# jrobine/actor-critic

Hardware: AMD Instinct MI355X
Metric: env-steps/sec (whole node) + ACKTR update ms, Breakout 84x84x4 (higher is better)
Workload: dtype fp32

## Files before the change

actor-critic_amd/csrc/convt2.hpp:

```cpp
#pragma once

#include "f16x2.hpp"
#include "gemm.hpp"

namespace acmi {

struct CT2 {
  static constexpr int CIN = 32, COUT = 64, OH = 9, OW = 9, PW = 10, L = 100;
  static constexpr int NKS = 16;
  static constexpr int STEP_BYTES = 4 * 2 * 1024;
  static constexpr int FRAG_BYTES = NKS * STEP_BYTES;
  static constexpr int BYTES = FRAG_BYTES + 4 * kAmaxWords;
  static constexpr int TILE = 128;
};

__device__ __forceinline__ void convt2_wmax_body(const float* w2, char* out, int b, int nb) {
  float m = 0.f;
  for (int i = b * 256 + threadIdx.x; i < 16 * CT2::CIN * CT2::COUT; i += nb * 256)
    m = fmaxf(m, fabsf(w2[i]));
  m = wave_max(m);
  if ((threadIdx.x & 63) == 0) amax_update(reinterpret_cast<unsigned*>(out + CT2::FRAG_BYTES), m);
}

__device__ __forceinline__ void convt2_prep_body(const float* w2, char* out, int blk) {
  const int g = blk * 256 + threadIdx.x;
  if (g >= CT2::NKS * 4 * 64) return;
  const int lane = g & 63, ph = (g >> 6) & 3, ks = g >> 8;
  const int py = ph >> 1, px = ph & 1, t = ks >> 2, a = t >> 1, b = t & 1;
  const int kh = py + 2 * a, kw = px + 2 * b;
  const int ci = lane & 31, co = 16 * (ks & 3) + 8 * (lane >> 5);
  const float* p = w2 + ((kh * 4 + kw) * CT2::CIN + ci) * CT2::COUT + co;
  const float sw = f16x2_scale_of_bits(reinterpret_cast<const unsigned*>(out + CT2::FRAG_BYTES));
  uint4 h, l;
  split2(p[0], p[1], sw, h.x, l.x);
  split2(p[2], p[3], sw, h.y, l.y);
  split2(p[4], p[5], sw, h.z, l.z);
  split2(p[6], p[7], sw, h.w, l.w);
  uint4* d = reinterpret_cast<uint4*>(out + (long long)ks * CT2::STEP_BYTES + ph * 2 * 1024) + lane;
  d[0] = h;
  d[64] = l;
}

template <bool GRAM, bool MASK = false, bool MIX = false>
__global__ __launch_bounds__(256) __attribute__((amdgpu_waves_per_eu(3)))
void convt2_kernel(const char* prep, const float* __restrict__ d2, const float* __restrict__ a1,
                   float* __restrict__ d1, int B, float* __restrict__ gpart, const unsigned* d2max,
                   unsigned* d1max, const float* __restrict__ d2b = nullptr, const unsigned* d2bmax = nullptr) {
  __shared__ __attribute__((aligned(16))) char lds[std::max(2 * CT2::STEP_BYTES, 4 * 32 * 36 * 4)];
  const int tid = threadIdx.x, lane = tid & 63, wave = tid >> 6;
  const int J = B * CT2::L;
  const int ctiles = (J + CT2::TILE - 1) / CT2::TILE;
  const int G = gridDim.x;
  const int gbase = MIX ? (ctiles + G - 1) / G * G : ctiles;
  const int ntiles = MIX ? gbase + ctiles : ctiles;
  auto valid_from = [&](int t) { return MIX && t >= ctiles && t < gbase ? t + G : t; };
  const int hl = lane >> 5;
  const float* zero = zero_run();
  const float sd_a = f16x2_scale_of_bits(d2max);
  const float sw = f16x2_scale_of_bits(reinterpret_cast<const unsigned*>(prep + CT2::FRAG_BYTES));
  const float inv_a = 1.f / (sw * sd_a);
  float sd_b = sd_a, inv_b = inv_a;
  if constexpr (MIX) {
    sd_b = f16x2_scale_of_bits(d2bmax);
    inv_b = 1.f / (sw * sd_b);
  }
  auto gram_tile = [&](int tile) { return MIX ? tile >= gbase : GRAM; };
  auto local_tile = [&](int tile) { return MIX && tile >= gbase ? tile - gbase : tile; };

  float d1am = 0.f;
  f32x16 gacc;
#pragma unroll
  for (int r = 0; r < 16; ++r) gacc[r] = 0.f;

  struct Col {
    bool ok;
    int n, Y, X;
    const float* dimg;
  };
  auto col_of = [&](int tile) {
    Col c;
    const int j = local_tile(tile) * CT2::TILE + 32 * wave + (lane & 31);
    c.ok = j < J;
    const int jj = c.ok ? j : 0;
    c.n = jj / CT2::L;
    const int sp = jj - c.n * CT2::L;
    c.Y = sp / CT2::PW;
    c.X = sp - c.Y * CT2::PW;
    c.dimg = (MIX && gram_tile(tile) ? d2b : d2) + (long long)c.n * (CT2::OH * CT2::OW * CT2::COUT);
    return c;
  };
  auto bload = [&](int ks, const Col& c, float4 (&x)[2]) {
    const int t = ks >> 2, a = t >> 1, b = t & 1;
    const int oy = c.Y - a, ox = c.X - b;
    const bool ok = c.ok & (oy >= 0) & (oy < CT2::OH) & (ox >= 0) & (ox < CT2::OW);
    const int oyc = max(oy, 0), oxc = max(ox, 0);
    const float* p = c.dimg + (oyc * CT2::OW + oxc) * CT2::COUT + 16 * (ks & 3) + 8 * hl;
    x[0] = *reinterpret_cast<const float4*>(ok ? p : zero);
    x[1] = *reinterpret_cast<const float4*>(ok ? p + 4 : zero);
  };
  uint4 ra0, ra1;
  auto afetch = [&](int ks) {
    const uint4* src = reinterpret_cast<const uint4*>(prep + (long long)ks * CT2::STEP_BYTES) + tid;
    ra0 = src[0];
    ra1 = src[256];
  };
  auto acommit = [&](int buf) {
    uint4* dst = reinterpret_cast<uint4*>(lds + buf * CT2::STEP_BYTES) + tid;
    dst[0] = ra0;
    dst[256] = ra1;
  };
  float4 bx0[2], bx1[2];
  const int first = valid_from(blockIdx.x);
  Col cur = col_of(min(first, ntiles - 1));
  afetch(0);
  bload(0, cur, bx0);

  for (int tile = first; tile < ntiles; tile = valid_from(tile + G)) {
    const Col nextc = col_of(min(valid_from(tile + G), ntiles - 1));
    const bool jok = cur.ok;
    const int n = cur.n, Y = cur.Y, X = cur.X;
    const bool gt = gram_tile(tile);
    const float sd = MIX && gt ? sd_b : sd_a, inv = MIX && gt ? inv_b : inv_a;
    acommit(0);
    __syncthreads();

    f32x16 acc[4];
#pragma unroll
    for (int p = 0; p < 4; ++p)
#pragma unroll
      for (int r = 0; r < 16; ++r) acc[p][r] = 0.f;

    auto step = [&](int ks, float4 (&cb)[2], float4 (&nb)[2]) {
      const int buf = ks & 1;
      const bool last = ks + 1 == CT2::NKS;
      afetch(last ? 0 : ks + 1);
      Col c;
      c.ok = last ? nextc.ok : cur.ok;
      c.Y = last ? nextc.Y : cur.Y;
      c.X = last ? nextc.X : cur.X;
      c.dimg = last ? nextc.dimg : cur.dimg;
      bload(last ? 0 : ks + 1, c, nb);
      __builtin_amdgcn_sched_barrier(0);
      f16x8 b[2];
      split2x8(cb[0], cb[1], sd, b[0], b[1]);
      const char* As = lds + buf * CT2::STEP_BYTES + lane * 16;
#pragma unroll
      for (int p = 0; p < 4; ++p) {
        f16x8 a[2];
#pragma unroll
        for (int q = 0; q < 2; ++q) a[q] = as_f16x8(*reinterpret_cast<const uint4*>(As + (p * 2 + q) * 1024));
        acc[p] = mfma_x2(a, b, acc[p]);
      }
      __builtin_amdgcn_sched_barrier(0);
      if (!last) acommit(buf ^ 1);
      __syncthreads();
    };
    for (int ks = 0; ks < CT2::NKS; ks += 2) {
      step(ks, bx0, bx1);
      step(ks + 1, bx1, bx0);
    }
    cur = nextc;
#pragma unroll
    for (int p = 0; p < 4; ++p)
#pragma unroll
      for (int r = 0; r < 16; ++r) acc[p][r] *= inv;

    float* scr = reinterpret_cast<float*>(lds) + wave * 32 * 36;
    if (!gt) {
      const int ri = 4 * (lane & 7), cj = lane >> 3;
      int pix[4];
      bool jok[4];
#pragma unroll
      for (int q = 0; q < 4; ++q) {
        const int j = local_tile(tile) * CT2::TILE + 32 * wave + cj + 8 * q;
        jok[q] = j < J;
        const int jj = jok[q] ? j : 0;
        const int nn = jj / CT2::L, sp = jj - nn * CT2::L;
        const int yy = sp / CT2::PW, xx = sp - yy * CT2::PW;
        pix[q] = (nn * 20 + 2 * yy) * 20 + 2 * xx;
      }
#pragma unroll
      for (int p = 0; p < 4; ++p) {
#pragma unroll
        for (int g = 0; g < 4; ++g)
          *reinterpret_cast<float4*>(scr + (lane & 31) * 36 + 8 * g + 4 * hl) =
              make_float4(acc[p][4 * g], acc[p][4 * g + 1], acc[p][4 * g + 2], acc[p][4 * g + 3]);
        __builtin_amdgcn_fence(__ATOMIC_RELEASE, "wavefront");
        __builtin_amdgcn_wave_barrier();
        __builtin_amdgcn_fence(__ATOMIC_ACQUIRE, "wavefront");
        const int dp = (p >> 1) * 20 + (p & 1);
        float4 v[4];
        uint32_t bits[4];
        float4 xa[4];
#pragma unroll
        for (int q = 0; q < 4; ++q) {
          v[q] = *reinterpret_cast<const float4*>(scr + (cj + 8 * q) * 36 + ri);
          const int px = pix[q] + dp;
          if constexpr (MASK) bits[q] = reinterpret_cast<const uint32_t*>(jok[q] ? a1 + px : zero)[0] >> ri;
          else xa[q] = *reinterpret_cast<const float4*>(jok[q] ? a1 + px * CT2::CIN + ri : zero);
        }
#pragma unroll
        for (int q = 0; q < 4; ++q) {
          float4 o;
          if constexpr (MASK) {
            o.x = (bits[q] & 1u) ? v[q].x : 0.f;
            o.y = (bits[q] & 2u) ? v[q].y : 0.f;
            o.z = (bits[q] & 4u) ? v[q].z : 0.f;
            o.w = (bits[q] & 8u) ? v[q].w : 0.f;
          } else {
            o.x = xa[q].x > 0.f ? v[q].x : 0.f;
            o.y = xa[q].y > 0.f ? v[q].y : 0.f;
            o.z = xa[q].z > 0.f ? v[q].z : 0.f;
            o.w = xa[q].w > 0.f ? v[q].w : 0.f;
          }
          if (jok[q]) {
            *reinterpret_cast<float4*>(d1 + (long long)(pix[q] + dp) * CT2::CIN + ri) = o;
            d1am = absmax4(d1am, o);
          }
        }
        __builtin_amdgcn_fence(__ATOMIC_RELEASE, "wavefront");
        __builtin_amdgcn_wave_barrier();
        __builtin_amdgcn_fence(__ATOMIC_ACQUIRE, "wavefront");
      }
    } else {
#pragma unroll
      for (int p = 0; p < 4; ++p) {
        const int py = p >> 1, px = p & 1;
        const long long pix = ((long long)n * 20 + 2 * Y + py) * 20 + 2 * X + px;
#pragma unroll
        for (int g = 0; g < 4; ++g) {
          const int ci = 8 * g + 4 * hl;
          float4 x;
          if constexpr (MASK) {
            const uint32_t b = *reinterpret_cast<const uint32_t*>(jok ? a1 + pix : zero) >> ci;
            x = make_float4((float)(b & 1u), (float)((b >> 1) & 1u), (float)((b >> 2) & 1u), (float)((b >> 3) & 1u));
          } else {
            x = *reinterpret_cast<const float4*>(jok ? a1 + pix * CT2::CIN + ci : zero);
          }
          const int c = lane & 31;
          scr[(ci + 0) * 36 + c] = x.x > 0.f ? acc[p][4 * g + 0] : 0.f;
          scr[(ci + 1) * 36 + c] = x.y > 0.f ? acc[p][4 * g + 1] : 0.f;
          scr[(ci + 2) * 36 + c] = x.z > 0.f ? acc[p][4 * g + 2] : 0.f;
          scr[(ci + 3) * 36 + c] = x.w > 0.f ? acc[p][4 * g + 3] : 0.f;
        }
        __builtin_amdgcn_wave_barrier();
#pragma unroll
        for (int h = 0; h < 2; ++h) {
          const float* rp = scr + (lane & 31) * 36 + 16 * h + 8 * hl;
          const float4 x0 = *reinterpret_cast<const float4*>(rp);
          const float4 x1 = *reinterpret_cast<const float4*>(rp + 4);
          uint4 hh, mm, ll;
          split3(x0.x, x0.y, hh.x, mm.x, ll.x);
          split3(x0.z, x0.w, hh.y, mm.y, ll.y);
          split3(x1.x, x1.y, hh.z, mm.z, ll.z);
          split3(x1.z, x1.w, hh.w, mm.w, ll.w);
          const bf16x8 f[3] = {__builtin_bit_cast(bf16x8, hh), __builtin_bit_cast(bf16x8, mm),
                               __builtin_bit_cast(bf16x8, ll)};
          gacc = mfma_x3(f, f, gacc);
        }
        __builtin_amdgcn_wave_barrier();
      }
    }
    __syncthreads();
  }

  if constexpr (MIX || !GRAM) amax_publish(d1max, d1am, lane);
  if constexpr (MIX || GRAM) {
    float* red = reinterpret_cast<float*>(lds);
    for (int w = 0; w < 4; ++w) {
      if (wave == w) {
#pragma unroll
        for (int r = 0; r < 16; ++r) {
          const int i = (r & 3) + 8 * (r >> 2) + 4 * hl, jc = lane & 31;
          red[i * 32 + jc] = (w ? red[i * 32 + jc] : 0.f) + gacc[r];
        }
      }
      __syncthreads();
    }
    float* out = gpart + (long long)blockIdx.x * 33 * 32;
    for (int e = tid; e < 32 * 32; e += 256) out[e] = red[e];
  }
}

struct CT2R {
  static constexpr int TEAMS = 3, THREADS = TEAMS * 256, WAVES = THREADS / 64;
  static constexpr int STORE_LD = 36, GRAM_LD = 20;
  static constexpr int WAVE_SCR = 4 * std::max(16 * STORE_LD, 32 * GRAM_LD);
  static constexpr int LDS_BYTES = CT2::FRAG_BYTES + WAVES * WAVE_SCR;
  static constexpr int MAX_TEAMS = 768;
};
static_assert(CT2R::LDS_BYTES <= 163840, "resident W2^T fragments + epilogue scratch exceed a CU's 160 KiB of LDS");
static_assert(4 * CT2R::WAVE_SCR >= 32 * 32 * 4, "a team's Gram sum red[32][32] aliases its four waves' scratch");
static_assert(CT2R::WAVE_SCR % 16 == 0 && CT2::FRAG_BYTES % (16 * 64) == 0, "16-byte LDS rows");

__device__ __attribute__((weak, aligned(16))) float kCt2ZeroPixel[CT2::COUT] = {};

template <bool GRAM, bool MASK>
__global__ __launch_bounds__(CT2R::THREADS)
void convt2_resident_kernel(const char* prep, const float* __restrict__ d2, const float* __restrict__ a1,
                            float* __restrict__ d1, int B, float* __restrict__ gpart, const unsigned* d2max,
                            unsigned* d1max, int G) {
  __shared__ __attribute__((aligned(16))) char lds[CT2R::LDS_BYTES];
  const int tid = threadIdx.x, lane = tid & 63;
  const int bwave = __builtin_amdgcn_readfirstlane(tid >> 6);
  const int wave = bwave & 3, team = bwave >> 2;
  const int J = B * CT2::L;
  const int ntiles = (J + CT2::TILE - 1) / CT2::TILE;
  const int v = CT2R::TEAMS * blockIdx.x + team;
  const bool active = v < G;
  const int hl = lane >> 5;
  const float* zero = zero_run();
  const float sd = f16x2_scale_of_bits(d2max);
  const float sw = f16x2_scale_of_bits(reinterpret_cast<const unsigned*>(prep + CT2::FRAG_BYTES));
  const float inv = 1.f / (sw * sd);

  float d1am = 0.f;
  f32x16 gacc;
#pragma unroll
  for (int r = 0; r < 16; ++r) gacc[r] = 0.f;

  struct Col {
    bool ok;
    int n, Y, X;
    const float* dimg;
  };
  auto col_of = [&](int tile) {
    Col c;
    const int j = tile * CT2::TILE + 32 * wave + (lane & 31);
    c.ok = j < J;
    const int jj = c.ok ? j : 0;
    c.n = jj / CT2::L;
    const int sp = jj - c.n * CT2::L;
    c.Y = sp / CT2::PW;
    c.X = sp - c.Y * CT2::PW;
    c.dimg = d2 + (long long)c.n * (CT2::OH * CT2::OW * CT2::COUT);
    return c;
  };
  auto tap_ptr = [&](int t, bool cok, int Y, int X, const float* dimg) {
    const int a = t >> 1, b = t & 1;
    const int oy = Y - a, ox = X - b;
    const bool ok = cok & (oy >= 0) & (oy < CT2::OH) & (ox >= 0) & (ox < CT2::OW);
    const int oyc = max(oy, 0), oxc = max(ox, 0);
    const float* p = dimg + (oyc * CT2::OW + oxc) * CT2::COUT;
    return (ok ? p : kCt2ZeroPixel) + 8 * hl;
  };
  auto bload = [&](const float* p, int cg, float4 (&x)[2]) {
    x[0] = *reinterpret_cast<const float4*>(p + 16 * cg);
    x[1] = *reinterpret_cast<const float4*>(p + 16 * cg + 4);
  };

  float4 bx0[2], bx1[2], bx2[2], bx3[2];
  Col cur = col_of(min(v, ntiles - 1));
  const float* pc = tap_ptr(0, cur.ok, cur.Y, cur.X, cur.dimg);
  bload(pc, 0, bx0);
  bload(pc, 1, bx1);

  {
    constexpr int RUNS = CT2::FRAG_BYTES / 16, PER = (RUNS + CT2R::THREADS - 1) / CT2R::THREADS;
    const uint4* src = reinterpret_cast<const uint4*>(prep);
    uint4* dst = reinterpret_cast<uint4*>(lds);
    uint4 r[PER];
#pragma unroll
    for (int k = 0; k < PER; ++k) r[k] = src[min(tid + CT2R::THREADS * k, RUNS - 1)];
#pragma unroll
    for (int k = 0; k < PER; ++k)
      if (tid + CT2R::THREADS * k < RUNS) dst[tid + CT2R::THREADS * k] = r[k];
  }
  __syncthreads();

  float* scr = reinterpret_cast<float*>(lds + CT2::FRAG_BYTES + bwave * CT2R::WAVE_SCR);
  const bool amax_per_tile = (G & (kAmaxSlots - 1)) != 0;
  auto publish_d1max = [&](int tile) {
    const float m = wave_max(d1am);
    if (d1max && lane == 0) {
      unsigned* q = d1max + kAmaxStride * (tile & (kAmaxSlots - 1));
      const unsigned u = __float_as_uint(m);
      if (u > __hip_atomic_load(q, __ATOMIC_RELAXED, __HIP_MEMORY_SCOPE_AGENT)) atomicMax(q, u);
    }
  };

  for (int tile = active ? v : ntiles; tile < ntiles; tile += G) {
    const Col nextc = col_of(min(tile + G, ntiles - 1));
    const bool jok = cur.ok;
    const int n = cur.n, Y = cur.Y, X = cur.X;

    f32x16 acc[4];
#pragma unroll
    for (int p = 0; p < 4; ++p)
#pragma unroll
      for (int r = 0; r < 16; ++r) acc[p][r] = 0.f;

    auto step = [&](const char* As, const float4 (&cb)[2], auto&& loads) {
      loads();
      __builtin_amdgcn_sched_barrier(0);
      auto aread = [&](int p, f16x8 (&a)[2]) {
#pragma unroll
        for (int q = 0; q < 2; ++q) a[q] = as_f16x8(*reinterpret_cast<const uint4*>(As + (p * 2 + q) * 1024));
      };
      f16x8 b[2], a0[2], a1[2];
      aread(0, a0);
      split2x8(cb[0], cb[1], sd, b[0], b[1]);
      aread(1, a1);
      acc[0] = mfma_x2(a0, b, acc[0]);
      aread(2, a0);
      acc[1] = mfma_x2(a1, b, acc[1]);
      aread(3, a1);
      acc[2] = mfma_x2(a0, b, acc[2]);
      acc[3] = mfma_x2(a1, b, acc[3]);
      __builtin_amdgcn_sched_group_barrier(0x100, 2, 0);
      __builtin_amdgcn_sched_group_barrier(0x002, 64, 0);
      __builtin_amdgcn_sched_group_barrier(0x100, 2, 0);
      __builtin_amdgcn_sched_group_barrier(0x008, 3, 0);
      __builtin_amdgcn_sched_group_barrier(0x100, 2, 0);
      __builtin_amdgcn_sched_group_barrier(0x008, 3, 0);
      __builtin_amdgcn_sched_group_barrier(0x100, 2, 0);
      __builtin_amdgcn_sched_group_barrier(0x008, 6, 0);
      __builtin_amdgcn_sched_barrier(0);
    };
#pragma unroll 1
    for (int t = 0; t < 4; ++t) {
      const bool wrap = t == 3;
      const float* pn = tap_ptr((t + 1) & 3, wrap ? nextc.ok : cur.ok, wrap ? nextc.Y : cur.Y,
                                wrap ? nextc.X : cur.X, wrap ? nextc.dimg : cur.dimg);
      const char* As = lds + t * (4 * CT2::STEP_BYTES) + lane * 16;
      step(As, bx0, [&] { bload(pc, 2, bx2); bload(pc, 3, bx3); });
      step(As + CT2::STEP_BYTES, bx1, [] {});
      step(As + 2 * CT2::STEP_BYTES, bx2, [&] { bload(pn, 0, bx0); bload(pn, 1, bx1); });
      step(As + 3 * CT2::STEP_BYTES, bx3, [] {});
      pc = pn;
    }
    cur = nextc;
#pragma unroll
    for (int p = 0; p < 4; ++p)
#pragma unroll
      for (int r = 0; r < 16; ++r) acc[p][r] *= inv;

    const int half = (lane >> 4) & 1;
    if constexpr (!GRAM) {
      const int ri = 4 * (lane & 7), cj = lane >> 3;
      int pix[4];
      bool qok[4];
#pragma unroll
      for (int q = 0; q < 4; ++q) {
        const int j = tile * CT2::TILE + 32 * wave + cj + 8 * q;
        qok[q] = j < J;
        const int jj = qok[q] ? j : 0;
        const int nn = jj / CT2::L, sp = jj - nn * CT2::L;
        const int yy = sp / CT2::PW, xx = sp - yy * CT2::PW;
        pix[q] = (nn * 20 + 2 * yy) * 20 + 2 * xx;
      }
#pragma unroll
      for (int p = 0; p < 4; ++p) {
        const int dp = (p >> 1) * 20 + (p & 1);
        uint32_t bits[4];
        float4 xa[4];
#pragma unroll
        for (int q = 0; q < 4; ++q) {
          const int px = pix[q] + dp;
          if constexpr (MASK) bits[q] = reinterpret_cast<const uint32_t*>(qok[q] ? a1 + px : zero)[0] >> ri;
          else xa[q] = *reinterpret_cast<const float4*>(qok[q] ? a1 + px * CT2::CIN + ri : zero);
        }
#pragma unroll
        for (int h = 0; h < 2; ++h) {
          if (half == h) {
#pragma unroll
            for (int g = 0; g < 4; ++g)
              *reinterpret_cast<float4*>(scr + (lane & 15) * CT2R::STORE_LD + 8 * g + 4 * hl) =
                  make_float4(acc[p][4 * g], acc[p][4 * g + 1], acc[p][4 * g + 2], acc[p][4 * g + 3]);
          }
          __builtin_amdgcn_fence(__ATOMIC_RELEASE, "wavefront");
          __builtin_amdgcn_wave_barrier();
          __builtin_amdgcn_fence(__ATOMIC_ACQUIRE, "wavefront");
#pragma unroll
          for (int q = 2 * h; q < 2 * h + 2; ++q) {
            const float4 x = *reinterpret_cast<const float4*>(scr + (cj + 8 * (q - 2 * h)) * CT2R::STORE_LD + ri);
            float4 o;
            if constexpr (MASK) {
              o.x = (bits[q] & 1u) ? x.x : 0.f;
              o.y = (bits[q] & 2u) ? x.y : 0.f;
              o.z = (bits[q] & 4u) ? x.z : 0.f;
              o.w = (bits[q] & 8u) ? x.w : 0.f;
            } else {
              o.x = xa[q].x > 0.f ? x.x : 0.f;
              o.y = xa[q].y > 0.f ? x.y : 0.f;
              o.z = xa[q].z > 0.f ? x.z : 0.f;
              o.w = xa[q].w > 0.f ? x.w : 0.f;
            }
            if (qok[q]) {
              *reinterpret_cast<float4*>(d1 + (long long)(pix[q] + dp) * CT2::CIN + ri) = o;
              d1am = absmax4(d1am, o);
            }
          }
          __builtin_amdgcn_fence(__ATOMIC_RELEASE, "wavefront");
          __builtin_amdgcn_wave_barrier();
          __builtin_amdgcn_fence(__ATOMIC_ACQUIRE, "wavefront");
        }
      }
      if (amax_per_tile) {
        publish_d1max(tile);
        d1am = 0.f;
      }
    } else {
#pragma unroll
      for (int p = 0; p < 4; ++p) {
        const int py = p >> 1, px = p & 1;
        const long long pix = ((long long)n * 20 + 2 * Y + py) * 20 + 2 * X + px;
#pragma unroll
        for (int g = 0; g < 4; ++g) {
          const int ci = 8 * g + 4 * hl;
          float4 x;
          if constexpr (MASK) {
            const uint32_t b = *reinterpret_cast<const uint32_t*>(jok ? a1 + pix : zero) >> ci;
            x = make_float4((float)(b & 1u), (float)((b >> 1) & 1u), (float)((b >> 2) & 1u), (float)((b >> 3) & 1u));
          } else {
            x = *reinterpret_cast<const float4*>(jok ? a1 + pix * CT2::CIN + ci : zero);
          }
          acc[p][4 * g + 0] = x.x > 0.f ? acc[p][4 * g + 0] : 0.f;
          acc[p][4 * g + 1] = x.y > 0.f ? acc[p][4 * g + 1] : 0.f;
          acc[p][4 * g + 2] = x.z > 0.f ? acc[p][4 * g + 2] : 0.f;
          acc[p][4 * g + 3] = x.w > 0.f ? acc[p][4 * g + 3] : 0.f;
        }
#pragma unroll
        for (int h = 0; h < 2; ++h) {
          if (half == h) {
#pragma unroll
            for (int r = 0; r < 16; ++r)
              scr[((r & 3) + 8 * (r >> 2) + 4 * hl) * CT2R::GRAM_LD + (lane & 15)] = acc[p][r];
          }
          __builtin_amdgcn_fence(__ATOMIC_RELEASE, "wavefront");
          __builtin_amdgcn_wave_barrier();
          __builtin_amdgcn_fence(__ATOMIC_ACQUIRE, "wavefront");
          const float* rp = scr + (lane & 31) * CT2R::GRAM_LD + 8 * hl;
          const float4 x0 = *reinterpret_cast<const float4*>(rp);
          const float4 x1 = *reinterpret_cast<const float4*>(rp + 4);
          uint4 hh, mm, ll;
          split3(x0.x, x0.y, hh.x, mm.x, ll.x);
          split3(x0.z, x0.w, hh.y, mm.y, ll.y);
          split3(x1.x, x1.y, hh.z, mm.z, ll.z);
          split3(x1.z, x1.w, hh.w, mm.w, ll.w);
          const bf16x8 f[3] = {__builtin_bit_cast(bf16x8, hh), __builtin_bit_cast(bf16x8, mm),
                               __builtin_bit_cast(bf16x8, ll)};
          gacc = mfma_x3(f, f, gacc);
          __builtin_amdgcn_fence(__ATOMIC_RELEASE, "wavefront");
          __builtin_amdgcn_wave_barrier();
          __builtin_amdgcn_fence(__ATOMIC_ACQUIRE, "wavefront");
        }
      }
    }
  }

  if constexpr (!GRAM) {
    if (active) publish_d1max(v);
  }
  __syncthreads();
  if constexpr (GRAM) {
    float* red = reinterpret_cast<float*>(lds + CT2::FRAG_BYTES + team * 4 * CT2R::WAVE_SCR);
    for (int w = 0; w < 4; ++w) {
      if (wave == w) {
#pragma unroll
        for (int r = 0; r < 16; ++r) {
          const int i = (r & 3) + 8 * (r >> 2) + 4 * hl, jc = lane & 31;
          red[i * 32 + jc] = (w ? red[i * 32 + jc] : 0.f) + gacc[r];
        }
      }
      __syncthreads();
    }
    if (active) {
      float* out = gpart + (long long)v * 33 * 32;
      for (int e = tid & 255; e < 32 * 32; e += 256) out[e] = red[e];
    }
  }
}

#ifndef ACMI_CT2_STORE_BLOCKS
#define ACMI_CT2_STORE_BLOCKS 0
#endif
inline int convt2_store_blocks(int B) {
  const int ntiles = (B * CT2::L + CT2::TILE - 1) / CT2::TILE;
  return ACMI_CT2_STORE_BLOCKS > 0 ? std::max(1, std::min(ntiles, ACMI_CT2_STORE_BLOCKS)) : ntiles;
}
inline int convt2_gram_blocks(int B) {
  const int ntiles = (B * CT2::L + CT2::TILE - 1) / CT2::TILE;
  return std::max(1, std::min(ntiles, 768));
}
inline int convt2_resident_teams(int B) { return convt2_gram_blocks(B); }
inline int convt2_resident_blocks(int B) { return (convt2_resident_teams(B) + CT2R::TEAMS - 1) / CT2R::TEAMS; }
static_assert(CT2R::MAX_TEAMS == 768 && CT2R::MAX_TEAMS % kAmaxSlots == 0, "teams = convt2_gram_blocks");
#ifndef ACMI_CT2R_MIN_TILES_STORE
#define ACMI_CT2R_MIN_TILES_STORE 2000
#endif
#ifndef ACMI_CT2R_MIN_TILES_GRAM
#define ACMI_CT2R_MIN_TILES_GRAM 2000
#endif
constexpr int kCt2ResidentMinTilesStore = ACMI_CT2R_MIN_TILES_STORE;
constexpr int kCt2ResidentMinTilesGram = ACMI_CT2R_MIN_TILES_GRAM;
inline bool convt2_resident_default(int B, bool gram) {
  const int ntiles = (B * CT2::L + CT2::TILE - 1) / CT2::TILE;
  return ntiles >= (gram ? kCt2ResidentMinTilesGram : kCt2ResidentMinTilesStore);
}

}
```

Before: 2.969 million.

## Reuse converted B fragments across horizontal taps via DPP lane shifts

The transposed-conv B operand for the second horizontal tap (b=1) is now built from the already converted fragments of the b=0 tap. The code shifts them across lanes with DPP row-rotate and row-broadcast, and fetches only one edge pixel per lane group. This halves the global loads and fp32-to-f16 split conversions per tile, replacing them with cheap cross-lane moves. The cost is more register pressure, a more intricate lane mapping that must be exactly right at column boundaries, and recomputing the column info each iteration.

```diff
diff --git a/actor-critic_amd/csrc/convt2.hpp b/actor-critic_amd/csrc/convt2.hpp
--- a/actor-critic_amd/csrc/convt2.hpp
+++ b/actor-critic_amd/csrc/convt2.hpp
@@ -348,10 +348,38 @@
     x[0] = *reinterpret_cast<const float4*>(p + 16 * cg);
     x[1] = *reinterpret_cast<const float4*>(p + 16 * cg + 4);
   };
+  const bool elane = (lane & 28) == 12;
+  auto edge_ptr = [&](int tile, int a) {
+    const int j0 = tile * CT2::TILE + 32 * wave;
+    const int n0 = j0 / CT2::L, sp = j0 - n0 * CT2::L;
+    const int Y0 = sp / CT2::PW, X0 = sp - Y0 * CT2::PW;
+    const int oy = Y0 - a;
+    const bool ok = elane & (j0 < J) & (X0 >= 1) & (oy >= 0) & (oy < CT2::OH);
+    const float* p = d2 + (long long)n0 * (CT2::OH * CT2::OW * CT2::COUT) +
+                     (max(oy, 0) * CT2::OW + max(X0 - 1, 0)) * CT2::COUT + 16 * (lane & 3);
+    return (ok ? p : kCt2ZeroPixel) + 8 * hl;
+  };
+  const bool lane32 = lane == 32;
+  auto shift = [&](auto cgc, const f16x8 (&k)[2], const f16x8 (&e)[2], f16x8 (&b)[2]) {
+    constexpr int ROR = 0x120 + 4 - decltype(cgc)::value;
+#pragma unroll
+    for (int q = 0; q < 2; ++q) {
+      const uint4 kw = __builtin_bit_cast(uint4, k[q]), ew = __builtin_bit_cast(uint4, e[q]);
+      auto sh = [&](uint32_t kx, uint32_t ex) {
+        const uint32_t ef = __builtin_amdgcn_update_dpp(0u, ex, ROR, 0xf, 0xf, false);
+        const uint32_t x = __builtin_amdgcn_update_dpp(ef, kx, 0x138, 0xf, 0xf, false);
+        return lane32 ? ef : x;
+      };
+      b[q] = as_f16x8(make_uint4(sh(kw.x, ew.x), sh(kw.y, ew.y), sh(kw.z, ew.z), sh(kw.w, ew.w)));
+    }
+  };
 
   float4 bx0[2], bx1[2], bx2[2], bx3[2];
-  Col cur = col_of(min(v, ntiles - 1));
-  const float* pc = tap_ptr(0, cur.ok, cur.Y, cur.X, cur.dimg);
+  const float* pc;
+  {
+    const Col c = col_of(min(v, ntiles - 1));
+    pc = tap_ptr(0, c.ok, c.Y, c.X, c.dimg);
+  }
   bload(pc, 0, bx0);
   bload(pc, 1, bx1);
 
@@ -380,26 +408,21 @@
   };
 
   for (int tile = active ? v : ntiles; tile < ntiles; tile += G) {
-    const Col nextc = col_of(min(tile + G, ntiles - 1));
-    const bool jok = cur.ok;
-    const int n = cur.n, Y = cur.Y, X = cur.X;
-
     f32x16 acc[4];
 #pragma unroll
     for (int p = 0; p < 4; ++p)
 #pragma unroll
       for (int r = 0; r < 16; ++r) acc[p][r] = 0.f;
 
-    auto step = [&](const char* As, const float4 (&cb)[2], auto&& loads) {
-      loads();
+    auto step = [&](const char* As, f16x8 (&b)[2], auto nvalu, auto&& make) {
       __builtin_amdgcn_sched_barrier(0);
       auto aread = [&](int p, f16x8 (&a)[2]) {
 #pragma unroll
         for (int q = 0; q < 2; ++q) a[q] = as_f16x8(*reinterpret_cast<const uint4*>(As + (p * 2 + q) * 1024));
       };
-      f16x8 b[2], a0[2], a1[2];
+      f16x8 a0[2], a1[2];
       aread(0, a0);
-      split2x8(cb[0], cb[1], sd, b[0], b[1]);
+      make();
       aread(1, a1);
       acc[0] = mfma_x2(a0, b, acc[0]);
       aread(2, a0);
@@ -408,7 +431,7 @@
       acc[2] = mfma_x2(a0, b, acc[2]);
       acc[3] = mfma_x2(a1, b, acc[3]);
       __builtin_amdgcn_sched_group_barrier(0x100, 2, 0);
-      __builtin_amdgcn_sched_group_barrier(0x002, 64, 0);
+      if constexpr (decltype(nvalu)::value > 0) __builtin_amdgcn_sched_group_barrier(0x002, decltype(nvalu)::value, 0);
       __builtin_amdgcn_sched_group_barrier(0x100, 2, 0);
       __builtin_amdgcn_sched_group_barrier(0x008, 3, 0);
       __builtin_amdgcn_sched_group_barrier(0x100, 2, 0);
@@ -417,24 +440,46 @@
       __builtin_amdgcn_sched_group_barrier(0x008, 6, 0);
       __builtin_amdgcn_sched_barrier(0);
     };
+    auto own = [&](const char* As, const float4 (&cb)[2], f16x8 (&k)[2]) {
+      step(As, k, std::integral_constant<int, 64>(), [&] { split2x8(cb[0], cb[1], sd, k[0], k[1]); });
+    };
+    auto shared = [&](const char* As, f16x8 (&b)[2]) { step(As, b, std::integral_constant<int, 0>(), [] {}); };
 #pragma unroll 1
-    for (int t = 0; t < 4; ++t) {
-      const bool wrap = t == 3;
-      const float* pn = tap_ptr((t + 1) & 3, wrap ? nextc.ok : cur.ok, wrap ? nextc.Y : cur.Y,
-                                wrap ? nextc.X : cur.X, wrap ? nextc.dimg : cur.dimg);
-      const char* As = lds + t * (4 * CT2::STEP_BYTES) + lane * 16;
-      step(As, bx0, [&] { bload(pc, 2, bx2); bload(pc, 3, bx3); });
-      step(As + CT2::STEP_BYTES, bx1, [] {});
-      step(As + 2 * CT2::STEP_BYTES, bx2, [&] { bload(pn, 0, bx0); bload(pn, 1, bx1); });
-      step(As + 3 * CT2::STEP_BYTES, bx3, [] {});
+    for (int a = 0; a < 2; ++a) {
+      const bool wrap = a == 1;
+      const Col c = col_of(wrap ? min(tile + G, ntiles - 1) : tile);
+      const float* pn = tap_ptr(wrap ? 0 : 2, c.ok, c.Y, c.X, c.dimg);
+      const char* As = lds + a * (8 * CT2::STEP_BYTES) + lane * 16;
+      f16x8 k0[2], k1[2], k2[2], k3[2], e[2], b[2];
+      float4 ex[2];
+      bload(pc, 2, bx2);
+      bload(pc, 3, bx3);
+      own(As, bx0, k0);
+      own(As + CT2::STEP_BYTES, bx1, k1);
+      bload(edge_ptr(tile, a), 0, ex);
+      own(As + 2 * CT2::STEP_BYTES, bx2, k2);
+      own(As + 3 * CT2::STEP_BYTES, bx3, k3);
+      split2x8(ex[0], ex[1], sd, e[0], e[1]);
+      shift(std::integral_constant<int, 0>(), k0, e, b);
+      shared(As + 4 * CT2::STEP_BYTES, b);
+      shift(std::integral_constant<int, 1>(), k1, e, b);
+      shared(As + 5 * CT2::STEP_BYTES, b);
+      shift(std::integral_constant<int, 2>(), k2, e, b);
+      bload(pn, 0, bx0);
+      bload(pn, 1, bx1);
+      shared(As + 6 * CT2::STEP_BYTES, b);
+      shift(std::integral_constant<int, 3>(), k3, e, b);
+      shared(As + 7 * CT2::STEP_BYTES, b);
       pc = pn;
     }
-    cur = nextc;
 #pragma unroll
     for (int p = 0; p < 4; ++p)
 #pragma unroll
       for (int r = 0; r < 16; ++r) acc[p][r] *= inv;
 
+    const Col cur = col_of(tile);
+    const bool jok = cur.ok;
+    const int n = cur.n, Y = cur.Y, X = cur.X;
     const int half = (lane >> 4) & 1;
     if constexpr (!GRAM) {
       const int ri = 4 * (lane & 7), cj = lane >> 3;
```

Result: no change. 2.967 million (-0.0%).
